# iKrishneel/fcn_object_detector

Hardware: AMD Instinct MI355X
Metric: frames/sec forward 448x448 @1 GPU; train imgs/sec @1/2/4/8 GPUs (higher is better)
Workload: dtype f32

## Files before the change

fcn_object_detector_amd/csrc/pointwise.hip:

```cpp
#include <float.h>
#include <math.h>

#include "common.h"

using namespace fcn;

namespace {

__device__ __forceinline__ float4 ld4(const float* p) { return *reinterpret_cast<const float4*>(p); }
__device__ __forceinline__ void st4(float* p, float4 v) { *reinterpret_cast<float4*>(p) = v; }

template <typename D>
__global__ __launch_bounds__(256) void nchw_to_nhwc_kernel(const float* __restrict__ src, D* __restrict__ dst,
                                                           int C, int HW, int dst_cstride, int dst_coffset, float shift) {
    __shared__ float tile[32][33];
    const int n = blockIdx.z;
    const int p0 = blockIdx.x * 32, c0 = blockIdx.y * 32;
    const int tx = threadIdx.x & 31, ty = threadIdx.x >> 5;
    const float* s = src + (size_t)n * C * HW;
    D* d = dst + (size_t)n * HW * dst_cstride;
    for (int i = ty; i < 32; i += 8) {
        const int c = c0 + i, p = p0 + tx;
        tile[i][tx] = (c < C && p < HW) ? s[(size_t)c * HW + p] : 0.f;
    }
// ... 7 lines not shown
template <typename S>
__global__ __launch_bounds__(256) void nhwc_to_nchw_kernel(const S* __restrict__ src, float* __restrict__ dst,
                                                           int C, int HW, int src_cstride, int src_coffset) {
    __shared__ float tile[32][33];
    const int n = blockIdx.z;
    const int p0 = blockIdx.x * 32, c0 = blockIdx.y * 32;
    const int tx = threadIdx.x & 31, ty = threadIdx.x >> 5;
    const S* s = src + (size_t)n * HW * src_cstride;
    float* d = dst + (size_t)n * C * HW;
    for (int i = ty; i < 32; i += 8) {
        const int p = p0 + i, c = c0 + tx;
        tile[i][tx] = (p < HW && c < C) ? (float)s[(size_t)p * src_cstride + src_coffset + c] : 0.f;
    }
    __syncthreads();
    for (int i = ty; i < 32; i += 8) {
        const int c = c0 + i, p = p0 + tx;
        if (c < C && p < HW) d[(size_t)c * HW + p] = tile[tx][i];
    }
}

__global__ __launch_bounds__(256) void nchw_to_nhwc4_kernel(const float* __restrict__ src, float* __restrict__ dst, int C, int HW, float shift) {
    const int n = blockIdx.y;
    const float* s = src + (size_t)n * C * HW;
    for (int p = blockIdx.x * blockDim.x + threadIdx.x; p < HW; p += gridDim.x * blockDim.x) {
        float4 v = make_float4(0.f, 0.f, 0.f, 0.f);
        v.x = s[p] + shift;
        if (C > 1) v.y = s[(size_t)HW + p] + shift;
        if (C > 2) v.z = s[2 * (size_t)HW + p] + shift;
        if (C > 3) v.w = s[3 * (size_t)HW + p] + shift;
        *reinterpret_cast<float4*>(dst + ((size_t)n * HW + p) * 4) = v;
    }
}

constexpr int kMaxLayoutBlobs = 8;
struct LayoutBlob { const float* src; float* dst; int C, HW, cstride, coffset, count, end; };
struct LayoutArgs { int n; LayoutBlob b[kMaxLayoutBlobs]; };
__global__ __launch_bounds__(256) void nhwc_to_nchw_multi_kernel(const LayoutArgs a) {
    const int total = a.b[a.n - 1].end;
    for (int i = blockIdx.x * blockDim.x + threadIdx.x; i < total; i += gridDim.x * blockDim.x) {
        int k = 0;
#pragma unroll
        for (int j = 0; j < kMaxLayoutBlobs - 1; ++j) k += (j + 1 < a.n && i >= a.b[j].end) ? 1 : 0;
        LayoutBlob q = a.b[0];
#pragma unroll
        for (int j = 1; j < kMaxLayoutBlobs; ++j)
            if (k == j) q = a.b[j];
        const int e = i - (q.end - q.count);
        const int p = e % q.HW, nc = e / q.HW;
        const int c = nc % q.C, n = nc / q.C;
        q.dst[e] = q.src[((size_t)n * q.HW + p) * q.cstride + q.coffset + c];
    }
}

template <bool VEC4, bool WITH_IDX>
__global__ __launch_bounds__(256) void maxpool_kernel(const float* __restrict__ x, float* __restrict__ y, int32_t* __restrict__ idx,
                                                      int N, int H, int W, int C, int x_cstride, int k, int stride, int pad,
                                                      int OH, int OW, int y_cstride, int y_coffset) {
    const int cg = VEC4 ? C / 4 : C;
    const long long total = (long long)N * OH * OW * cg;
    for (long long t = (long long)blockIdx.x * blockDim.x + threadIdx.x; t < total; t += (long long)gridDim.x * blockDim.x) {
        const int g = (int)(t % cg);
        long long pix = t / cg;
        const int ox = (int)(pix % OW);
        pix /= OW;
        const int oy = (int)(pix % OH);
        const int n = (int)(pix / OH);
        int hs = oy * stride - pad, ws = ox * stride - pad;
        const int he = min(hs + k, H), we = min(ws + k, W);
        hs = max(hs, 0);
        ws = max(ws, 0);
        const float* xb = x + (size_t)n * H * W * x_cstride + (VEC4 ? g * 4 : g);
        const size_t o = ((size_t)(n * OH + oy) * OW + ox);
        if (VEC4) {
            float4 m = make_float4(-FLT_MAX, -FLT_MAX, -FLT_MAX, -FLT_MAX);
            int4 mi = make_int4(-1, -1, -1, -1);
            if (k == 3) {
                const int y0 = oy * stride - pad, x0 = ox * stride - pad;
                float4 v[9];
                int id[9];
                bool in[9];
#pragma unroll
                for (int r = 0; r < 3; ++r) {
                    const int iy = min(max(y0 + r, 0), H - 1);
// ... 1105 lines not shown
        _Float16* dp = dst + (size_t)pix * dst_cstride + dst_coffset;
        if (!VEC) {
            dp[c] = sp[c];
        } else if (c * 8 + 8 <= C) {
            *(h8_t*)(dp + c * 8) = *(const h8_t*)(sp + c * 8);
        } else {
            const h8_t v = *(const h8_t*)(sp + c * 8);
#pragma unroll
            for (int e = 0; e < 7; ++e)
                if (c * 8 + e < C) dp[c * 8 + e] = v[e];
        }
    }
}

extern "C" {

int fcn_nchw_to_nhwc_f32(const float* src, float* dst, int N, int C, int H, int W, int dst_cstride, int dst_coffset, float shift,
                         fcn_stream_t s) {
    FCN_REQUIRE(src && dst && N > 0 && C > 0 && H > 0 && W > 0, FCN_E_ARG, "nchw_to_nhwc: bad args");
    FCN_REQUIRE(dst_coffset >= 0 && dst_cstride >= dst_coffset + C, FCN_E_ARG, "nchw_to_nhwc: slice exceeds dst_cstride");
    FCN_REQUIRE(N <= 65535, FCN_E_UNSUPPORTED, "nchw_to_nhwc: batch too large");
    const int HW = H * W;
    if (C <= 4 && dst_cstride == 4 && dst_coffset == 0 && ((uintptr_t)dst & 15) == 0) {
        hipLaunchKernelGGL(nchw_to_nhwc4_kernel, dim3(cdiv(HW, 256) < 4096 ? cdiv(HW, 256) : 4096, N), dim3(256), 0, as_stream(s), src, dst, C, HW, shift);
        FCN_LAUNCH_CHECK("nchw_to_nhwc4");
        return 0;
    }
    dim3 grid(cdiv(HW, 32), cdiv(C, 32), N);
    hipLaunchKernelGGL(nchw_to_nhwc_kernel<float>, grid, dim3(256), 0, as_stream(s), src, dst, C, HW, dst_cstride, dst_coffset, shift);
    FCN_LAUNCH_CHECK("nchw_to_nhwc");
    return 0;
}

int fcn_nhwc_to_nchw_multi_f32(const fcn_layout_desc* h_descs, int n, fcn_stream_t s) {
    FCN_REQUIRE(h_descs && n > 0 && n <= kMaxLayoutBlobs, FCN_E_ARG, "nhwc_to_nchw_multi: 1..%d blobs", kMaxLayoutBlobs);
    LayoutArgs a;
    a.n = n;
    long long end = 0;
    for (int i = 0; i < kMaxLayoutBlobs; ++i) {
        const fcn_layout_desc& d = h_descs[i < n ? i : n - 1];
        if (i < n) {
            FCN_REQUIRE(d.src && d.dst && d.N > 0 && d.C > 0 && d.H > 0 && d.W > 0, FCN_E_ARG, "nhwc_to_nchw_multi: bad blob %d", i);
            FCN_REQUIRE(d.src_coffset >= 0 && d.src_cstride >= d.src_coffset + d.C, FCN_E_ARG, "nhwc_to_nchw_multi: slice of blob %d exceeds its stride", i);
            end += (long long)d.N * d.C * d.H * d.W;
            FCN_REQUIRE(end < (1ll << 30), FCN_E_UNSUPPORTED, "nhwc_to_nchw_multi: meant for small blobs");
        }
        LayoutBlob& b = a.b[i];
        b.src = d.src; b.dst = d.dst; b.C = d.C; b.HW = d.H * d.W; b.cstride = d.src_cstride; b.coffset = d.src_coffset;
        b.count = i < n ? d.N * d.C * d.H * d.W : 0;
        b.end = (int)end;
    }
    const int blocks = cdiv(end, 256) < 2048 ? cdiv(end, 256) : 2048;
    hipLaunchKernelGGL(nhwc_to_nchw_multi_kernel, dim3(blocks), dim3(256), 0, as_stream(s), a);
    FCN_LAUNCH_CHECK("nhwc_to_nchw_multi");
    return 0;
}

int fcn_nchw_f32_to_nhwc_f16(const float* src, void* dst, int N, int C, int H, int W, int dst_cstride, int dst_coffset, float shift,
                             fcn_stream_t s) {
    FCN_REQUIRE(src && dst && N > 0 && C > 0 && H > 0 && W > 0, FCN_E_ARG, "nchw_to_nhwc_f16: bad args");
    FCN_REQUIRE(dst_coffset >= 0 && dst_cstride >= dst_coffset + C, FCN_E_ARG, "nchw_to_nhwc_f16: slice exceeds dst_cstride");
    FCN_REQUIRE(N <= 65535, FCN_E_UNSUPPORTED, "nchw_to_nhwc_f16: batch too large");
    const int HW = H * W;
    dim3 grid(cdiv(HW, 32), cdiv(C, 32), N);
    hipLaunchKernelGGL(nchw_to_nhwc_kernel<_Float16>, grid, dim3(256), 0, as_stream(s), src, reinterpret_cast<_Float16*>(dst), C, HW, dst_cstride,
                       dst_coffset, shift);
    FCN_LAUNCH_CHECK("nchw_to_nhwc_f16");
    return 0;
}

int fcn_nhwc_f16_to_nchw_f32(const void* src, float* dst, int N, int C, int H, int W, int src_cstride, int src_coffset, fcn_stream_t s) {
    FCN_REQUIRE(src && dst && N > 0 && C > 0 && H > 0 && W > 0, FCN_E_ARG, "nhwc_f16_to_nchw: bad args");
    FCN_REQUIRE(src_coffset >= 0 && src_cstride >= src_coffset + C, FCN_E_ARG, "nhwc_f16_to_nchw: slice exceeds src_cstride");
    FCN_REQUIRE(N <= 65535, FCN_E_UNSUPPORTED, "nhwc_f16_to_nchw: batch too large");
    const int HW = H * W;
    dim3 grid(cdiv(HW, 32), cdiv(C, 32), N);
    hipLaunchKernelGGL(nhwc_to_nchw_kernel<_Float16>, grid, dim3(256), 0, as_stream(s), reinterpret_cast<const _Float16*>(src), dst, C, HW,
                       src_cstride, src_coffset);
    FCN_LAUNCH_CHECK("nhwc_f16_to_nchw");
    return 0;
}

int fcn_nhwc_to_nchw_f32(const float* src, float* dst, int N, int C, int H, int W, int src_cstride, int src_coffset, fcn_stream_t s) {
    FCN_REQUIRE(src && dst && N > 0 && C > 0 && H > 0 && W > 0, FCN_E_ARG, "nhwc_to_nchw: bad args");
    FCN_REQUIRE(src_coffset >= 0 && src_cstride >= src_coffset + C, FCN_E_ARG, "nhwc_to_nchw: slice exceeds src_cstride");
    FCN_REQUIRE(N <= 65535, FCN_E_UNSUPPORTED, "nhwc_to_nchw: batch too large");
    const int HW = H * W;
// ... 412 lines not shown
```

fcn_object_detector_amd/csrc/runtime.hip:

```cpp
#include <stdarg.h>

#include "common.h"

namespace fcn {

char* err_buf() {
    static thread_local char buf[512] = {0};
    return buf;
}

int set_err(int code, const char* fmt, ...) {
    va_list ap;
    va_start(ap, fmt);
    vsnprintf(err_buf(), 512, fmt, ap);
    va_end(ap);
    return code;
}

}

using namespace fcn;

extern "C" {

// ... 20 lines not shown
    FCN_HIP(hipGetDevice(&dev));
    hipDeviceProp_t prop;
    FCN_HIP(hipGetDeviceProperties(&prop, dev));
    snprintf(h_buf, len, "%s (%s, %d CUs)", prop.name, prop.gcnArchName, prop.multiProcessorCount);
    return 0;
}

int fcn_device_sync(void) {
    FCN_HIP(hipDeviceSynchronize());
    return 0;
}

int fcn_malloc(void** p, size_t bytes) {
    FCN_REQUIRE(p, FCN_E_ARG, "fcn_malloc: null");
    if (bytes == 0) bytes = 16;
    FCN_HIP(hipMalloc(p, bytes));
    return 0;
}

int fcn_free(void* p) {
    if (p) FCN_HIP(hipFree(p));
    return 0;
}

int fcn_host_malloc(void** h_p, size_t bytes) {
    FCN_REQUIRE(h_p, FCN_E_ARG, "fcn_host_malloc: null");
    if (bytes == 0) bytes = 16;
    FCN_HIP(hipHostMalloc(h_p, bytes, hipHostMallocDefault));
    return 0;
}

int fcn_host_free(void* h_p) {
    if (h_p) FCN_HIP(hipHostFree(h_p));
    return 0;
}

int fcn_memset_async(void* p, int value, size_t bytes, fcn_stream_t s) {
    FCN_REQUIRE(p || bytes == 0, FCN_E_ARG, "fcn_memset_async: null");
    if (bytes) FCN_HIP(hipMemsetAsync(p, value, bytes, as_stream(s)));
    return 0;
}

int fcn_memcpy_h2d_async(void* dst, const void* h_src, size_t bytes, fcn_stream_t s) {
    FCN_REQUIRE((dst && h_src) || bytes == 0, FCN_E_ARG, "fcn_memcpy_h2d_async: null");
    if (bytes) FCN_HIP(hipMemcpyAsync(dst, h_src, bytes, hipMemcpyHostToDevice, as_stream(s)));
    return 0;
}

int fcn_memcpy_d2h_async(void* h_dst, const void* src, size_t bytes, fcn_stream_t s) {
    FCN_REQUIRE((h_dst && src) || bytes == 0, FCN_E_ARG, "fcn_memcpy_d2h_async: null");
    if (bytes) FCN_HIP(hipMemcpyAsync(h_dst, src, bytes, hipMemcpyDeviceToHost, as_stream(s)));
    return 0;
}

int fcn_memcpy_d2d_async(void* dst, const void* src, size_t bytes, fcn_stream_t s) {
    FCN_REQUIRE((dst && src) || bytes == 0, FCN_E_ARG, "fcn_memcpy_d2d_async: null");
    if (bytes) FCN_HIP(hipMemcpyAsync(dst, src, bytes, hipMemcpyDeviceToDevice, as_stream(s)));
    return 0;
}

int fcn_stream_create(fcn_stream_t* s) {
    FCN_REQUIRE(s, FCN_E_ARG, "fcn_stream_create: null");
    hipStream_t st;
    FCN_HIP(hipStreamCreateWithFlags(&st, hipStreamNonBlocking));
    *s = st;
    return 0;
// ... 80 lines not shown
```

fcn_object_detector_amd/engine.py:

```python
from __future__ import annotations

import ctypes as C
import os
import threading
from typing import Callable, Dict, List, Optional, Sequence, Tuple

import numpy as np

from . import lib as L
from .netspec import Layer, NetSpec, kernel_stride_pad

F32 = np.float32


def _r4(c: int) -> int:
    return (c + 3) // 4 * 4


def _ra(c: int, esize: int) -> int:
    eps = 16 // esize
    return (c + eps - 1) // eps * eps


class DeviceBuffer:
# ... 9 lines not shown

    def free(self) -> None:
        if getattr(self, "ptr", 0):
            try:
                L.load().fcn_free(self.ptr)
            finally:
                self.ptr = 0

    def __del__(self):
        try:
            self.free()
        except Exception:
            pass


class DevView:

    __slots__ = ("ptr", "nbytes")

    def __init__(self, ptr: int, nbytes: int):
        self.ptr, self.nbytes = int(ptr), int(nbytes)


class PinnedArray:

    def __init__(self, shape: Tuple[int, ...]):
        n = int(np.prod(shape)) if len(shape) else 1
        p = C.c_void_p()
        L.call("fcn_host_malloc", C.byref(p), max(n, 1) * 4)
        self.ptr = int(p.value)
        buf = (C.c_float * max(n, 1)).from_address(self.ptr)
        self.array = np.frombuffer(buf, dtype=F32, count=n).reshape(shape)
        self.array[...] = 0

    def free(self) -> None:
        if getattr(self, "ptr", 0):
            self.array = None
            try:
                L.load().fcn_host_free(self.ptr)
            finally:
                self.ptr = 0

    def __del__(self):
        try:
            self.free()
        except Exception:
            pass


class Blob:

    def __init__(self, name: str, shape: Tuple[int, ...]):
        self.name = name
        self.shape = tuple(shape)
        self.buf: Optional[DeviceBuffer] = None
        self.coffset = 0
        self.cstride = 0
        self.esize = 4
        self.lazy_shift = 0.0
        self.upload_shift = 0.0
        self.host: Optional[np.ndarray] = None
        self.pinned: Optional[PinnedArray] = None
        self.host_valid = False
        self.is_input = False

    @property
# ... 32 lines not shown
                 share_params: Optional["Engine"] = None, score_outputs: bool = False):
        if dtype not in ("f32", "f16"):
            raise ValueError("dtype must be 'f32' or 'f16'")
        if share_params is not None and (dtype != "f32" or share_params.f16):
            raise NotImplementedError("share_params: only between float32 engines (a half-float engine packs its weights differently)")
        self._share_from = share_params
        self.shared_layers: set = set()
        self.score_outputs = bool(score_outputs)
        self.score_acc: Dict[str, DeviceBuffer] = {}
        self.graph_score: Optional[int] = None
        if dtype == "f16" and spec.phase != "TEST":
            raise NotImplementedError("the half-float path is inference only (BASELINE configs[4])")
        self.dtype, self.f16 = dtype, dtype == "f16"
        self.spec = spec
        self.device = device
        self.fuse = fuse
        self.group_convs = group_convs
        self.autotune = autotune
        self._chosen_cfgs: Dict[str, int] = {}
        self._tune_from = tune_from
        self._tune_max_lds = int(tune_max_lds_kb if tune_max_lds_kb is not None else os.environ.get("FCN_TUNE_MAX_LDS_KB", "160")) * 1024
        self._tune_streams = int(tune_streams if tune_streams is not None else os.environ.get("FCN_TUNE_STREAMS", "1"))
        L.call("fcn_init", device)
        sp = C.c_void_p()
        L.call("fcn_stream_create", C.byref(sp))
        self.stream = int(sp.value)
        self.lock = threading.RLock()
        self.shapes = spec.infer(data_shapes)
        self.blobs: Dict[str, Blob] = {}
        self.params_host: Dict[str, List[np.ndarray]] = {}
        self.params_dev: Dict[str, List[DevView]] = {}
        self.ops: List[Op] = []
        self.graph_io: Optional[int] = None
        self.graph_core: Optional[int] = None
        self._staging: Dict[str, DeviceBuffer] = {}
        self._keep: List[object] = []
        self._conv_layer_meta: Dict[str, dict] = {}
        self._group_workspaces: List[DeviceBuffer] = []
        self.aux_dev: Dict[str, DeviceBuffer] = {}
        self._lazy_blob_ops: Dict[str, List[Op]] = {}
        self.loss_blobs: Dict[str, float] = {}
        self.device_fed: set = set()
        self.dropout_seed = 0
        self.dropout_index_offset = 0
        self.inputs = spec.data_tops()
        self.outputs = [b for b in spec.output_blobs() if b in self.shapes]
        self._plan_buffers()
        self._alloc_params(params)
        self._build_ops()
        self._release_tuning_resources()

    def _plan_buffers(self) -> None:
        spec = self.spec
        producers: Dict[str, List[Layer]] = {}
        consumers: Dict[str, List[Layer]] = {}
        for l in spec.layers:
            for t in l.tops:
                producers.setdefault(t, []).append(l)
            for b in l.bottoms:
                consumers.setdefault(b, []).append(l)
        self.producers, self.consumers = producers, consumers
        data_tops = set(self.inputs)
        self._half_inputs: Dict[str, Tuple[str, float]] = {}
        if self.f16 and self.fuse and os.environ.get("FCN_F16_IMAGE", "1") != "0":
            for d in data_tops:
                cons = consumers.get(d, [])
# ... 1124 lines not shown
                out.append(Op("tconv", l.name, lambda st: L.check(lib.fcn_tconv2d_f32(C.byref(plan), st)),
                              2.0 * n * h * w * c * co * k * k, 4.0 * (xb.pixels * c + yb.pixels * co)))
                return out
            if halves:
                if xb.esize != 2 or xb.coffset % 8:
                    raise NotImplementedError("f16 engine: Deconvolution %s from a float32 blob / an unaligned channel slice" % l.name)
                out.append(Op("deconv", l.name, lambda st: L.check(lib.fcn_deconv_depthwise_fwd_f16(
                    xb.ptr, wdev, bdev, yb.buf.ptr, n, h, w, c, xb.cstride, k, s, pad, oh, ow, yb.cstride, yb.coffset,
                    1 if yb.esize == 4 else 0, st)),
                    2.0 * yb.pixels * c * (k / s) ** 2, float(xb.esize * xb.pixels + yb.esize * yb.pixels) * c))
                return out
            out.append(Op("deconv", l.name, lambda st: L.check(lib.fcn_deconv_depthwise_fwd_f32(
                xb.ptr, wdev, bdev, yb.buf.ptr, n, h, w, c, xb.cstride, k, s, pad, oh, ow, yb.cstride, yb.coffset, st)),
                2.0 * yb.pixels * c * (k / s) ** 2, 4.0 * (xb.pixels + yb.pixels) * c))
        else:
            raise NotImplementedError("layer type %r (layer %s) has no forward kernel yet" % (t, l.name))
        return out

    def _stage(self, name: str) -> DeviceBuffer:
        st = self._staging.get(name)
        if st is None:
            b = self.blobs[name]
            st = DeviceBuffer(max(int(np.prod(b.shape)) if b.shape else 1, 1) * 4, zero=False)
            self._staging[name] = st
        return st

    def host_array(self, name: str) -> np.ndarray:
        b = self.blobs[name]
        if b.host is None:
            b.pinned = PinnedArray(b.shape)
            b.host = b.pinned.array
        return b.host

    def _upload_copy(self, name: str, stream: Optional[int]) -> None:
        b = self.blobs[name]
        host = self.host_array(name)
        dst = b.ptr if len(b.shape) != 4 else self._stage(name).ptr
        L.check(L.load().fcn_memcpy_h2d_async(dst, host.ctypes.data, host.nbytes, stream))

    def _upload_convert(self, name: str, stream: Optional[int]) -> None:
        b = self.blobs[name]
        if len(b.shape) != 4:
            return
        lib = L.load()
        n, c, h, w = b.shape
        st = self._stage(name)
        if b.esize == 2:
            L.check(lib.fcn_nchw_f32_to_nhwc_f16(st.ptr, b.buf.ptr, n, c, h, w, b.cstride, b.coffset, b.upload_shift, stream))
        else:
            L.check(lib.fcn_nchw_to_nhwc_f32(st.ptr, b.buf.ptr, n, c, h, w, b.cstride, b.coffset, b.upload_shift, stream))

    def _download_convert(self, name: str, stream: Optional[int]) -> None:
        b = self.blobs[name]
        if len(b.shape) != 4:
            return
        lib = L.load()
        n, c, h, w = b.shape
        st = self._stage(name)
        if b.esize == 2:
            L.check(lib.fcn_nhwc_f16_to_nchw_f32(b.buf.ptr, st.ptr, n, c, h, w, b.cstride, b.coffset, stream))
        else:
            L.check(lib.fcn_nhwc_to_nchw_f32(b.buf.ptr, st.ptr, n, c, h, w, b.cstride, b.coffset, stream))

    def _download_convert_all(self, stream: Optional[int]) -> None:
        multi = [nm for nm in self.outputs if len(self.blobs[nm].shape) == 4 and self.blobs[nm].esize == 4]
        if 2 <= len(multi) <= 8:
            if not hasattr(self, "_multi_descs"):
                arr = (L.LayoutDesc * len(multi))()
                for d, nm in zip(arr, multi):
                    b = self.blobs[nm]
                    n, c, h, w = b.shape
                    d.src, d.dst, d.N, d.C, d.H, d.W, d.src_cstride, d.src_coffset = b.buf.ptr, self._stage(nm).ptr, n, c, h, w, b.cstride, b.coffset
                self._multi_descs = arr
            L.check(L.load().fcn_nhwc_to_nchw_multi_f32(self._multi_descs, len(multi), stream))
        else:
            multi = []
        for nm in self.outputs:
            if nm not in multi:
                self._download_convert(nm, stream)

    def _download_copy(self, name: str, stream: Optional[int]) -> None:
        b = self.blobs[name]
        host = self.host_array(name)
        src = b.ptr if len(b.shape) != 4 else self._stage(name).ptr
        L.check(L.load().fcn_memcpy_d2h_async(host.ctypes.data, src, host.nbytes, stream))

    def _enqueue_upload(self, name: str, stream: Optional[int]) -> None:
        self._upload_copy(name, stream)
        self._upload_convert(name, stream)

    def _enqueue_download(self, name: str, stream: Optional[int]) -> None:
        self._download_convert(name, stream)
        self._download_copy(name, stream)

    def read_blob(self, name: str) -> np.ndarray:
        with self.lock:
            L.call("fcn_init", self.device)
            b = self.blobs[name]
            host = self.host_array(name)
            if not b.host_valid:
                for op in self._lazy_blob_ops.get(name, ()):
                    op.run(self.stream)
                self._enqueue_download(name, self.stream)
                L.call("fcn_stream_sync", self.stream)
                if b.lazy_shift:
                    host += F32(b.lazy_shift)
                b.host_valid = True
            return host

    LABEL_TOPS = ("coverage-label", "bbox-label", "size-block", "obj-block", "coverage-block")

    def set_targets(self, rects: Sequence[Sequence[Sequence[int]]], labels: Sequence[Sequence[int]], stride: int,
                    iou_thresh: float = 0.1, tops: Sequence[str] = LABEL_TOPS) -> None:
        fg = self.blobs[tops[0]]
# ... 66 lines not shown
            if self.graph_score is not None:
                L.call("fcn_graph_launch", self.graph_score, self.stream)
            else:
                for nm in self.inputs:
                    if nm not in self.device_fed:
                        self._upload_convert(nm, self.stream)
                self.run_ops(self.stream)
            for b in self.blobs.values():
                b.host_valid = False
            self.score_forwards += 1

    def score_read(self) -> Dict[str, np.ndarray]:
        with self.lock:
            out = {nm: np.empty(self.blobs[nm].shape, F32) for nm in self.outputs}
            for nm, a in out.items():
                L.call("fcn_memcpy_d2h_async", a.ctypes.data, self.score_acc[nm].ptr, a.nbytes, self.stream)
            L.call("fcn_stream_sync", self.stream)
            return out

    def run_ops(self, stream: Optional[int]) -> None:
        for op in self.ops:
            op.run(stream)

    def _capture(self, with_io: bool, download: bool = True) -> int:
        if with_io:
            for nm in list(self.inputs) + list(self.outputs):
                self.host_array(nm)
                if len(self.blobs[nm].shape) == 4:
                    self._stage(nm)
        if not getattr(self, "_warm", False):
            self.run_ops(self.stream)
            L.call("fcn_stream_sync", self.stream)
            self._warm = True
        if with_io and not getattr(self, "_warm_io", False):
            for nm in self.inputs:
                if nm not in self.device_fed:
                    self._enqueue_upload(nm, self.stream)
            self._download_convert_all(self.stream)
            for nm in self.outputs:
                self._download_copy(nm, self.stream)
            L.call("fcn_stream_sync", self.stream)
            self._warm_io = True
        L.call("fcn_graph_begin", self.stream)
        try:
            if with_io:
                for nm in self.inputs:
                    if nm not in self.device_fed:
                        self._upload_convert(nm, self.stream)
            self.run_ops(self.stream)
            if with_io and download:
                self._download_convert_all(self.stream)
        finally:
            g = C.c_void_p()
            L.call("fcn_graph_end", self.stream, C.byref(g))
        return int(g.value)

    def _launch_io(self) -> None:
        if self.graph_io is None:
            self.graph_io = self._capture(with_io=True)
        for nm in self.inputs:
            if nm not in self.device_fed:
                self._upload_copy(nm, self.stream)
        L.call("fcn_graph_launch", self.graph_io, self.stream)
        for nm in self.outputs:
            self._download_copy(nm, self.stream)

    def forward(self, use_graph: bool = True) -> Dict[str, np.ndarray]:
        use_graph = use_graph and os.environ.get("FCN_NO_GRAPH", "0") in ("", "0")
        with self.lock:
            L.call("fcn_init", self.device)
            for nm in self.inputs:
                self.host_array(nm)
            for nm in self.outputs:
                self.host_array(nm)
            if use_graph:
                self._launch_io()
            else:
                for nm in self.inputs:
                    if nm not in self.device_fed:
                        self._enqueue_upload(nm, self.stream)
                self.run_ops(self.stream)
                for nm in self.outputs:
                    self._enqueue_download(nm, self.stream)
            L.call("fcn_stream_sync", self.stream)
            for b in self.blobs.values():
                b.host_valid = False
            out = {}
            for nm in self.outputs:
                b = self.blobs[nm]
                if b.lazy_shift:
                    b.host += F32(b.lazy_shift)
                b.host_valid = True
                out[nm] = b.host
            for nm in self.inputs:
                self.blobs[nm].host_valid = nm not in self.device_fed
            return out

    def forward_begin(self) -> None:
# ... 256 lines not shown
```

fcn_object_detector_amd/lib.py:

```python
from __future__ import annotations

import ctypes as C
import os
import threading
from typing import Optional

_HERE = os.path.dirname(os.path.abspath(__file__))
LIB_PATH = os.environ.get("FCN_LIB_PATH") or os.path.join(_HERE, "libfcnhip.so")


class FcnLibraryError(RuntimeError):
    pass


class FcnError(RuntimeError):
    def __init__(self, code: int, msg: str):
        super().__init__("libfcnhip error %d: %s" % (code, msg))
        self.code = code


class ConvDesc(C.Structure):
    _fields_ = [
        ("x", C.c_void_p), ("w", C.c_void_p), ("bias", C.c_void_p), ("y", C.c_void_p), ("y2", C.c_void_p),
        ("N", C.c_int32), ("H", C.c_int32), ("W", C.c_int32), ("Cin", C.c_int32), ("x_cstride", C.c_int32),
# ... 58 lines not shown
    _fields_ = [("w_offset", C.c_uint64), ("wt_offset", C.c_uint64), ("Cout", C.c_int32), ("kh", C.c_int32), ("kw", C.c_int32),
                ("Cin", C.c_int32), ("Cin4", C.c_int32), ("Cout4", C.c_int32)]


class DetectParams(C.Structure):
    _fields_ = [
        ("num_classes", C.c_int32), ("gy", C.c_int32), ("gx", C.c_int32), ("cell_w", C.c_int32), ("cell_h", C.c_int32),
        ("cvg_cstride", C.c_int32), ("cvg_coffset", C.c_int32), ("box_cstride", C.c_int32), ("box_coffset", C.c_int32),
        ("prob_thresh", C.c_float), ("group_thresh", C.c_int32), ("eps", C.c_double), ("min_height", C.c_int32),
        ("round_mode", C.c_int32), ("max_out", C.c_int32),
    ]


CONV_RELU, CONV_SIGMOID2, CONV_ACCUM, CONV_OUT_F32, CONV_F16, CONV_OUT_F16, CONV_MASK = 1, 2, 4, 8, 16, 32, 64
CONV_IMAGE_ONES = 128
ELT_PROD, ELT_SUM, ELT_MAX = 0, 1, 2
SOLVER_KINDS = {"SGD": 0, "NESTEROV": 1, "ADAGRAD": 2, "RMSPROP": 3, "ADADELTA": 4, "ADAM": 5}
REG_L2, REG_L1 = 0, 1
RECT_ROUND_NEAREST_EVEN, RECT_ROUND_TRUNCATE = 0, 1

_vp, _i, _f, _d, _sz = C.c_void_p, C.c_int, C.c_float, C.c_double, C.c_size_t

PROTOTYPES = {
    "fcn_abi_version": (_i, []),
    "fcn_last_error_string": (C.c_char_p, []),
    "fcn_device_count": (_i, [C.POINTER(_i)]),
    "fcn_init": (_i, [_i]),
    "fcn_device_name": (_i, [C.c_char_p, _i]),
    "fcn_device_sync": (_i, []),
    "fcn_malloc": (_i, [C.POINTER(_vp), _sz]),
    "fcn_free": (_i, [_vp]),
    "fcn_host_malloc": (_i, [C.POINTER(_vp), _sz]),
    "fcn_host_free": (_i, [_vp]),
    "fcn_memset_async": (_i, [_vp, _i, _sz, _vp]),
    "fcn_memcpy_h2d_async": (_i, [_vp, _vp, _sz, _vp]),
    "fcn_memcpy_d2h_async": (_i, [_vp, _vp, _sz, _vp]),
    "fcn_memcpy_d2d_async": (_i, [_vp, _vp, _sz, _vp]),
    "fcn_stream_create": (_i, [C.POINTER(_vp)]),
    "fcn_stream_destroy": (_i, [_vp]),
    "fcn_stream_sync": (_i, [_vp]),
    "fcn_event_create": (_i, [C.POINTER(_vp)]),
    "fcn_event_destroy": (_i, [_vp]),
    "fcn_event_record": (_i, [_vp, _vp]),
    "fcn_event_sync": (_i, [_vp]),
    "fcn_event_elapsed_ms": (_i, [_vp, _vp, C.POINTER(_f)]),
    "fcn_graph_begin": (_i, [_vp]),
    "fcn_graph_end": (_i, [_vp, C.POINTER(_vp)]),
    "fcn_graph_launch": (_i, [_vp, _vp]),
    "fcn_graph_destroy": (_i, [_vp]),
    "fcn_nchw_to_nhwc_f32": (_i, [_vp, _vp, _i, _i, _i, _i, _i, _i, _f, _vp]),
    "fcn_nhwc_to_nchw_f32": (_i, [_vp, _vp, _i, _i, _i, _i, _i, _i, _vp]),
    "fcn_nhwc_to_nchw_multi_f32": (_i, [C.POINTER(LayoutDesc), _i, _vp]),
    "fcn_conv2d_fwd_f32": (_i, [C.POINTER(ConvDesc), _vp]),
    "fcn_conv2d_group_workspace_bytes": (_sz, [_i]),
    "fcn_conv2d_num_configs": (_i, []),
    "fcn_conv2d_first_layer_config": (_i, []),
    "fcn_conv2d_config_lds_bytes": (_i, [_i]),
    "fcn_conv2d_config_waves_k": (_i, [_i]),
    "fcn_conv2d_group_prepare": (_i, [C.POINTER(ConvDesc), _i, _vp, _i, C.POINTER(ConvGroup)]),
    "fcn_conv2d_group_prepare_fused": (_i, [C.POINTER(ConvDesc), _i, C.POINTER(PoolDesc), _i, _vp, _i, C.POINTER(ConvGroup)]),
    "fcn_conv2d_fwd_group_f32": (_i, [C.POINTER(ConvGroup), _vp]),
    "fcn_conv2d_group_release": (_i, [_vp]),
    "fcn_conv2d_tail_scratch_bytes": (C.c_size_t, [C.POINTER(ConvTail)]),
    "fcn_conv2d_tail_arrive_bytes": (C.c_size_t, [C.POINTER(ConvTail)]),
    "fcn_conv2d_group_attach_tail": (_i, [_vp, C.POINTER(ConvTail)]),
    "fcn_maxpool_fwd_f32": (_i, [_vp, _vp, _vp] + [_i] * 12 + [_vp]),
    "fcn_avepool_fwd_f32": (_i, [_vp, _vp] + [_i] * 12 + [_vp]),
    "fcn_lrn_fwd_f32": (_i, [_vp, _vp, _vp, _i, _i, _i, _i, _i, _f, _f, _f, _vp]),
    "fcn_maxpool_lrn5_fwd_f32": (_i, [_vp, _vp] + [_i] * 12 + [_f, _f, _f, _vp]),
    "fcn_maxpool_lrn5_fwd_f16": (_i, [_vp, _vp] + [_i] * 12 + [_f, _f, _f, _vp]),
    "fcn_maxpool_lrn5_conv1x1_fwd_f32": (_i, [_vp] + [_i] * 10 + [_f, _f, _f, _vp, _vp, _i, _i, _vp, _i, _i, _vp]),
    "fcn_maxpool_lrn5_conv1x1_fwd_f16": (_i, [_vp] + [_i] * 10 + [_f, _f, _f, _vp, _vp, _i, _i, _vp, _i, _i, _vp]),
    "fcn_relu_fwd_f32": (_i, [_vp, _vp, _sz, _f, _vp]),
    "fcn_sigmoid_fwd_f32": (_i, [_vp, _vp, _sz, _vp]),
    "fcn_power_fwd_f32": (_i, [_vp, _vp, _sz, _f, _f, _f, _vp]),
    "fcn_eltwise_fwd_f32": (_i, [_vp, _vp, _vp, _sz, _i, _f, _f, _vp]),
    "fcn_copy_channels_f32": (_i, [_vp, _vp, _i, _i, _i, _i, _i, _i, _vp]),
    "fcn_deconv_depthwise_fwd_f32": (_i, [_vp, _vp, _vp, _vp] + [_i] * 12 + [_vp]),
    "fcn_preprocess_bgr8": (_i, [_vp, _i, _i, _vp, _i, _i, _i, _f, _vp, _vp]),
    "fcn_detect_workspace_bytes": (_sz, [C.POINTER(DetectParams), _i]),
    "fcn_detect_decode_group": (_i, [_vp, _vp, _i, _sz, _sz, C.POINTER(DetectParams), _vp, _vp, _vp, _vp, _vp]),
    "fcn_score_masks_workspace_bytes": (_sz, [_i, _i, _i, _i]),
    "fcn_score_masks": (_i, [_vp, _i, _i, _i, _i, _i, _i, _vp, _f, _vp, _i, _i, _vp, _vp, _vp]),
    "fcn_gen_targets": (_i, [_vp, _vp, _vp, _i, _i, _i, _i, _i, _d, _vp, _vp, _vp, _vp, _vp, _vp]),
    "fcn_gen_targets_nhwc": (_i, [_vp, _vp, _vp, _i, _i, _i, _i, _i, _d, _vp, _i, _vp, _vp, _vp, _vp, _i, _vp]),
# ... 119 lines not shown
```

include/fcnhip.h:

```cpp
#ifndef FCNHIP_H_
#define FCNHIP_H_

#include <stddef.h>
#include <stdint.h>

#ifdef __cplusplus
extern "C" {
#endif

#define FCN_ABI_VERSION 1

#define FCN_E_ARG       1
#define FCN_E_ALIGN     2
#define FCN_E_UNSUPPORTED 3
#define FCN_E_STATE     4
#define FCN_E_CAPACITY  5

typedef void* fcn_stream_t;
typedef void* fcn_event_t;
typedef void* fcn_graph_t;
typedef void* fcn_comm_t;

int  fcn_abi_version(void);
const char* fcn_last_error_string(void);
int  fcn_device_count(int* count);
int  fcn_init(int device);
int  fcn_device_name(char* h_buf, int len);
int  fcn_device_sync(void);
int  fcn_malloc(void** p, size_t bytes);
int  fcn_free(void* p);
int  fcn_host_malloc(void** h_p, size_t bytes);
int  fcn_host_free(void* h_p);
int  fcn_memset_async(void* p, int value, size_t bytes, fcn_stream_t s);
int  fcn_memcpy_h2d_async(void* dst, const void* h_src, size_t bytes, fcn_stream_t s);
int  fcn_memcpy_d2h_async(void* h_dst, const void* src, size_t bytes, fcn_stream_t s);
int  fcn_memcpy_d2d_async(void* dst, const void* src, size_t bytes, fcn_stream_t s);
int  fcn_stream_create(fcn_stream_t* s);
int  fcn_stream_destroy(fcn_stream_t s);
int  fcn_stream_sync(fcn_stream_t s);
int  fcn_event_create(fcn_event_t* e);
int  fcn_event_destroy(fcn_event_t e);
int  fcn_event_record(fcn_event_t e, fcn_stream_t s);
int  fcn_event_sync(fcn_event_t e);
int  fcn_event_elapsed_ms(fcn_event_t start, fcn_event_t stop, float* h_ms);
int  fcn_stream_wait_event(fcn_stream_t s, fcn_event_t e);
int  fcn_graph_begin(fcn_stream_t s);
int  fcn_graph_end(fcn_stream_t s, fcn_graph_t* g);
int  fcn_graph_launch(fcn_graph_t g, fcn_stream_t s);
int  fcn_graph_destroy(fcn_graph_t g);

int  fcn_nchw_to_nhwc_f32(const float* src, float* dst, int N, int C, int H, int W,
                          int dst_cstride, int dst_coffset, float shift, fcn_stream_t s);
int  fcn_nhwc_to_nchw_f32(const float* src, float* dst, int N, int C, int H, int W,
                          int src_cstride, int src_coffset, fcn_stream_t s);
typedef struct fcn_layout_desc {
    const float* src;
    float* dst;
    int32_t N, C, H, W, src_cstride, src_coffset;
} fcn_layout_desc;
int  fcn_nhwc_to_nchw_multi_f32(const fcn_layout_desc* h_descs, int n, fcn_stream_t s);

#define FCN_CONV_RELU      1
#define FCN_CONV_SIGMOID2  2
#define FCN_CONV_ACCUM     4
#define FCN_CONV_MASK     64
#define FCN_CONV_IMAGE_ONES 128
#define FCN_CONV_OUT_F32   8
#define FCN_CONV_OUT_F16  32
#define FCN_CONV_F16      16
typedef struct fcn_conv_desc {
    const float* x;
    const float* w;
    const float* bias;
    float*       y;
    float*       y2;
    int32_t N, H, W, Cin, x_cstride;
    int32_t Cout, kh, kw, pad, stride, OH, OW;
    int32_t y_cstride, y_coffset, y2_cstride, y2_coffset;
    int32_t flags;
    float   in_shift;
} fcn_conv_desc;
int  fcn_conv2d_fwd_f32(const fcn_conv_desc* h_desc, fcn_stream_t s);
typedef struct fcn_conv_group {
    void*   d_probs;
    int32_t n;
    int32_t cfg;
    int32_t total_tiles;
} fcn_conv_group;
size_t fcn_conv2d_group_workspace_bytes(int n);
int  fcn_conv2d_num_configs(void);
int  fcn_conv2d_first_layer_config(void);
typedef struct fcn_conv_tail {
    int32_t n;
// ... 243 lines not shown
```

Baseline: 4237.

## Write outputs directly into pinned host memory via zero-copy kernels

Adds zero-copy I/O. The layout-conversion kernels now read the input frame from, or write outputs into, mapped pinned host memory through device pointers. This removes the separate staging buffers and the d2h/h2d memcpy steps around the captured graph. Output stores to host memory use nontemporal writes, with blob starts padded to 64 elements, and an optional vectorised host-read input kernel uses a small grid. The risk is that PCIe-latency-bound kernel stores run inside the graph and could slow it, and that the graph must be recaptured if the pinned buffers change.

```diff
diff --git a/fcn_object_detector_amd/csrc/pointwise.hip b/fcn_object_detector_amd/csrc/pointwise.hip
--- a/fcn_object_detector_amd/csrc/pointwise.hip
+++ b/fcn_object_detector_amd/csrc/pointwise.hip
@@ -63,23 +63,60 @@
     }
 }
 
+constexpr int kHostGroups = 2;
+constexpr int kHostGridMax = 64;
+typedef float f32x4 __attribute__((ext_vector_type(4)));
+template <int C>
+__global__ __launch_bounds__(256) void nchw_to_nhwc4_from_host_kernel(const float* __restrict__ src, float* __restrict__ dst, int HW, float shift) {
+    const int n = blockIdx.y;
+    const int groups = HW / 4, stride = gridDim.x * blockDim.x;
+    const f32x4* s = reinterpret_cast<const f32x4*>(src + (size_t)n * C * HW);
+    f32x4* d = reinterpret_cast<f32x4*>(dst + (size_t)n * HW * 4);
+    for (int g0 = blockIdx.x * blockDim.x + threadIdx.x; g0 < groups; g0 += stride * kHostGroups) {
+        f32x4 v[kHostGroups][C];
+#pragma unroll
+        for (int u = 0; u < kHostGroups; ++u) {
+            const int g = g0 + u * stride;
+#pragma unroll
+            for (int c = 0; c < C; ++c) v[u][c] = g < groups ? __builtin_nontemporal_load(s + (size_t)c * groups + g) : f32x4{0.f, 0.f, 0.f, 0.f};
+        }
+#pragma unroll
+        for (int u = 0; u < kHostGroups; ++u) {
+            const int g = g0 + u * stride;
+            if (g < groups) {
+#pragma unroll
+                for (int j = 0; j < 4; ++j) {
+                    f32x4 o = {0.f, 0.f, 0.f, 0.f};
+#pragma unroll
+                    for (int c = 0; c < C; ++c) o[c] = v[u][c][j] + shift;
+                    d[(size_t)g * 4 + j] = o;
+                }
+            }
+        }
+    }
+}
+
 constexpr int kMaxLayoutBlobs = 8;
-struct LayoutBlob { const float* src; float* dst; int C, HW, cstride, coffset, count, end; };
+struct LayoutBlob { const float* src; float* dst; int C, HW, cstride, coffset, start, end; };
 struct LayoutArgs { int n; LayoutBlob b[kMaxLayoutBlobs]; };
+template <bool TO_HOST>
 __global__ __launch_bounds__(256) void nhwc_to_nchw_multi_kernel(const LayoutArgs a) {
     const int total = a.b[a.n - 1].end;
     for (int i = blockIdx.x * blockDim.x + threadIdx.x; i < total; i += gridDim.x * blockDim.x) {
         int k = 0;
 #pragma unroll
-        for (int j = 0; j < kMaxLayoutBlobs - 1; ++j) k += (j + 1 < a.n && i >= a.b[j].end) ? 1 : 0;
+        for (int j = 0; j < kMaxLayoutBlobs - 1; ++j) k += (j + 1 < a.n && i >= a.b[j + 1].start) ? 1 : 0;
         LayoutBlob q = a.b[0];
 #pragma unroll
         for (int j = 1; j < kMaxLayoutBlobs; ++j)
             if (k == j) q = a.b[j];
-        const int e = i - (q.end - q.count);
+        if (i >= q.end) continue;
+        const int e = i - q.start;
         const int p = e % q.HW, nc = e / q.HW;
         const int c = nc % q.C, n = nc / q.C;
-        q.dst[e] = q.src[((size_t)n * q.HW + p) * q.cstride + q.coffset + c];
+        const float v = q.src[((size_t)n * q.HW + p) * q.cstride + q.coffset + c];
+        if (TO_HOST) __builtin_nontemporal_store(v, q.dst + e);
+        else q.dst[e] = v;
     }
 }
 
@@ -1251,27 +1288,54 @@
     return 0;
 }
 
-int fcn_nhwc_to_nchw_multi_f32(const fcn_layout_desc* h_descs, int n, fcn_stream_t s) {
+static int nhwc_to_nchw_multi(const fcn_layout_desc* h_descs, int n, bool to_host, fcn_stream_t s) {
     FCN_REQUIRE(h_descs && n > 0 && n <= kMaxLayoutBlobs, FCN_E_ARG, "nhwc_to_nchw_multi: 1..%d blobs", kMaxLayoutBlobs);
     LayoutArgs a;
     a.n = n;
     long long end = 0;
     for (int i = 0; i < kMaxLayoutBlobs; ++i) {
         const fcn_layout_desc& d = h_descs[i < n ? i : n - 1];
+        LayoutBlob& b = a.b[i];
+        b.src = d.src; b.dst = d.dst; b.C = d.C; b.HW = d.H * d.W; b.cstride = d.src_cstride; b.coffset = d.src_coffset;
+        if (to_host) end = (end + 63) / 64 * 64;
+        b.start = (int)end;
         if (i < n) {
             FCN_REQUIRE(d.src && d.dst && d.N > 0 && d.C > 0 && d.H > 0 && d.W > 0, FCN_E_ARG, "nhwc_to_nchw_multi: bad blob %d", i);
             FCN_REQUIRE(d.src_coffset >= 0 && d.src_cstride >= d.src_coffset + d.C, FCN_E_ARG, "nhwc_to_nchw_multi: slice of blob %d exceeds its stride", i);
             end += (long long)d.N * d.C * d.H * d.W;
             FCN_REQUIRE(end < (1ll << 30), FCN_E_UNSUPPORTED, "nhwc_to_nchw_multi: meant for small blobs");
         }
-        LayoutBlob& b = a.b[i];
-        b.src = d.src; b.dst = d.dst; b.C = d.C; b.HW = d.H * d.W; b.cstride = d.src_cstride; b.coffset = d.src_coffset;
-        b.count = i < n ? d.N * d.C * d.H * d.W : 0;
         b.end = (int)end;
     }
     const int blocks = cdiv(end, 256) < 2048 ? cdiv(end, 256) : 2048;
-    hipLaunchKernelGGL(nhwc_to_nchw_multi_kernel, dim3(blocks), dim3(256), 0, as_stream(s), a);
+    if (to_host) hipLaunchKernelGGL(nhwc_to_nchw_multi_kernel<true>, dim3(blocks), dim3(256), 0, as_stream(s), a);
+    else hipLaunchKernelGGL(nhwc_to_nchw_multi_kernel<false>, dim3(blocks), dim3(256), 0, as_stream(s), a);
     FCN_LAUNCH_CHECK("nhwc_to_nchw_multi");
+    return 0;
+}
+
+int fcn_nhwc_to_nchw_multi_f32(const fcn_layout_desc* h_descs, int n, fcn_stream_t s) { return nhwc_to_nchw_multi(h_descs, n, false, s); }
+
+int fcn_nhwc_to_nchw_multi_f32_to_host(const fcn_layout_desc* h_descs, int n, fcn_stream_t s) { return nhwc_to_nchw_multi(h_descs, n, true, s); }
+
+int fcn_nchw_to_nhwc_f32_from_host(const float* src, float* dst, int N, int C, int H, int W, int dst_cstride, int dst_coffset, float shift,
+                                   fcn_stream_t s) {
+    FCN_REQUIRE(src && dst && N > 0 && C > 0 && H > 0 && W > 0, FCN_E_ARG, "nchw_to_nhwc_from_host: bad args");
+    FCN_REQUIRE(dst_coffset >= 0 && dst_cstride >= dst_coffset + C, FCN_E_ARG, "nchw_to_nhwc_from_host: slice exceeds dst_cstride");
+    FCN_REQUIRE(N <= 65535, FCN_E_UNSUPPORTED, "nchw_to_nhwc_from_host: batch too large");
+    const int HW = H * W;
+    if (!(C <= 4 && dst_cstride == 4 && dst_coffset == 0 && HW % 4 == 0 && (((uintptr_t)src | (uintptr_t)dst) & 15) == 0))
+        return fcn_nchw_to_nhwc_f32(src, dst, N, C, H, W, dst_cstride, dst_coffset, shift, s);
+    int blocks = cdiv(HW / 4, 256 * kHostGroups);
+    if (blocks > kHostGridMax) blocks = cdiv(blocks, cdiv(blocks, kHostGridMax));
+    const dim3 grid(blocks, N);
+    switch (C) {
+        case 1: hipLaunchKernelGGL(nchw_to_nhwc4_from_host_kernel<1>, grid, dim3(256), 0, as_stream(s), src, dst, HW, shift); break;
+        case 2: hipLaunchKernelGGL(nchw_to_nhwc4_from_host_kernel<2>, grid, dim3(256), 0, as_stream(s), src, dst, HW, shift); break;
+        case 3: hipLaunchKernelGGL(nchw_to_nhwc4_from_host_kernel<3>, grid, dim3(256), 0, as_stream(s), src, dst, HW, shift); break;
+        default: hipLaunchKernelGGL(nchw_to_nhwc4_from_host_kernel<4>, grid, dim3(256), 0, as_stream(s), src, dst, HW, shift); break;
+    }
+    FCN_LAUNCH_CHECK("nchw_to_nhwc4_from_host");
     return 0;
 }
 
diff --git a/fcn_object_detector_amd/csrc/runtime.hip b/fcn_object_detector_amd/csrc/runtime.hip
--- a/fcn_object_detector_amd/csrc/runtime.hip
+++ b/fcn_object_detector_amd/csrc/runtime.hip
@@ -76,6 +76,12 @@
 
 int fcn_host_free(void* h_p) {
     if (h_p) FCN_HIP(hipHostFree(h_p));
+    return 0;
+}
+
+int fcn_host_device_ptr(void* h_p, void** d_p) {
+    FCN_REQUIRE(h_p && d_p, FCN_E_ARG, "fcn_host_device_ptr: null");
+    FCN_HIP(hipHostGetDevicePointer(d_p, h_p, 0));
     return 0;
 }
 
diff --git a/fcn_object_detector_amd/engine.py b/fcn_object_detector_amd/engine.py
--- a/fcn_object_detector_amd/engine.py
+++ b/fcn_object_detector_amd/engine.py
@@ -65,6 +65,14 @@
         buf = (C.c_float * max(n, 1)).from_address(self.ptr)
         self.array = np.frombuffer(buf, dtype=F32, count=n).reshape(shape)
         self.array[...] = 0
+        self._device_ptr = 0
+
+    def device_ptr(self) -> int:
+        if not self._device_ptr:
+            p = C.c_void_p()
+            L.call("fcn_host_device_ptr", self.ptr, C.byref(p))
+            self._device_ptr = int(p.value)
+        return self._device_ptr
 
     def free(self) -> None:
         if getattr(self, "ptr", 0):
@@ -163,6 +171,8 @@
         self.params_dev: Dict[str, List[DevView]] = {}
         self.ops: List[Op] = []
         self.graph_io: Optional[int] = None
+        self._direct: frozenset = frozenset()
+        self._graph_io_hosts: Dict[str, int] = {}
         self.graph_core: Optional[int] = None
         self._staging: Dict[str, DeviceBuffer] = {}
         self._keep: List[object] = []
@@ -1353,7 +1363,18 @@
             b.host = b.pinned.array
         return b.host
 
+    def _direct_io_names(self) -> frozenset:
+        level = os.environ.get("FCN_ZERO_COPY_IO", "1") or "0"
+        if level not in ("0", "1", "2"):
+            raise ValueError("FCN_ZERO_COPY_IO must be 0 (staged), 1 (outputs written to host memory) or 2 (and the frame read from it)")
+        plain = lambda b: len(b.shape) == 4 and b.esize == 4
+        ins = [nm for nm in self.inputs if nm not in self.device_fed and plain(self.blobs[nm])] if level == "2" else []
+        outs = [nm for nm in self.outputs if plain(self.blobs[nm]) and not self.blobs[nm].lazy_shift and nm not in self.inputs]
+        return frozenset(ins + (outs if level != "0" and len(outs) <= 8 else []))
+
     def _upload_copy(self, name: str, stream: Optional[int]) -> None:
+        if name in self._direct:
+            return
         b = self.blobs[name]
         host = self.host_array(name)
         dst = b.ptr if len(b.shape) != 4 else self._stage(name).ptr
@@ -1365,6 +1386,9 @@
             return
         lib = L.load()
         n, c, h, w = b.shape
+        if name in self._direct:
+            L.check(lib.fcn_nchw_to_nhwc_f32_from_host(b.pinned.device_ptr(), b.buf.ptr, n, c, h, w, b.cstride, b.coffset, b.upload_shift, stream))
+            return
         st = self._stage(name)
         if b.esize == 2:
             L.check(lib.fcn_nchw_f32_to_nhwc_f16(st.ptr, b.buf.ptr, n, c, h, w, b.cstride, b.coffset, b.upload_shift, stream))
@@ -1384,23 +1408,32 @@
             L.check(lib.fcn_nhwc_to_nchw_f32(b.buf.ptr, st.ptr, n, c, h, w, b.cstride, b.coffset, stream))
 
     def _download_convert_all(self, stream: Optional[int]) -> None:
-        multi = [nm for nm in self.outputs if len(self.blobs[nm].shape) == 4 and self.blobs[nm].esize == 4]
+        def descs(names, dst):
+            arr = (L.LayoutDesc * len(names))()
+            for d, nm in zip(arr, names):
+                b = self.blobs[nm]
+                n, c, h, w = b.shape
+                d.src, d.dst, d.N, d.C, d.H, d.W, d.src_cstride, d.src_coffset = b.buf.ptr, dst(nm), n, c, h, w, b.cstride, b.coffset
+            return arr
+        direct = [nm for nm in self.outputs if nm in self._direct]
+        if direct:
+            if getattr(self, "_direct_descs", None) is None:
+                self._direct_descs = descs(direct, lambda nm: self.blobs[nm].pinned.device_ptr())
+            L.check(L.load().fcn_nhwc_to_nchw_multi_f32_to_host(self._direct_descs, len(direct), stream))
+        multi = [nm for nm in self.outputs if nm not in direct and len(self.blobs[nm].shape) == 4 and self.blobs[nm].esize == 4]
         if 2 <= len(multi) <= 8:
             if not hasattr(self, "_multi_descs"):
-                arr = (L.LayoutDesc * len(multi))()
-                for d, nm in zip(arr, multi):
-                    b = self.blobs[nm]
-                    n, c, h, w = b.shape
-                    d.src, d.dst, d.N, d.C, d.H, d.W, d.src_cstride, d.src_coffset = b.buf.ptr, self._stage(nm).ptr, n, c, h, w, b.cstride, b.coffset
-                self._multi_descs = arr
+                self._multi_descs = descs(multi, lambda nm: self._stage(nm).ptr)
             L.check(L.load().fcn_nhwc_to_nchw_multi_f32(self._multi_descs, len(multi), stream))
         else:
             multi = []
         for nm in self.outputs:
-            if nm not in multi:
+            if nm not in multi and nm not in direct:
                 self._download_convert(nm, stream)
 
     def _download_copy(self, name: str, stream: Optional[int]) -> None:
+        if name in self._direct:
+            return
         b = self.blobs[name]
         host = self.host_array(name)
         src = b.ptr if len(b.shape) != 4 else self._stage(name).ptr
@@ -1533,38 +1566,54 @@
             self.run_ops(self.stream)
             L.call("fcn_stream_sync", self.stream)
             self._warm = True
-        if with_io and not getattr(self, "_warm_io", False):
+        self._direct = self._direct_io_names() if with_io and download else frozenset()
+        try:
+            for nm in self._direct:
+                self.blobs[nm].pinned.device_ptr()
+            warm = "_warm_io_direct" if self._direct else "_warm_io"
+            if with_io and not getattr(self, warm, False):
+                for nm in self.inputs:
+                    if nm not in self.device_fed:
+                        self._enqueue_upload(nm, self.stream)
+                self._download_convert_all(self.stream)
+                for nm in self.outputs:
+                    self._download_copy(nm, self.stream)
+                L.call("fcn_stream_sync", self.stream)
+                setattr(self, warm, True)
+            L.call("fcn_graph_begin", self.stream)
+            try:
+                if with_io:
+                    for nm in self.inputs:
+                        if nm not in self.device_fed:
+                            self._upload_convert(nm, self.stream)
+                self.run_ops(self.stream)
+                if with_io and download:
+                    self._download_convert_all(self.stream)
+            finally:
+                g = C.c_void_p()
+                L.call("fcn_graph_end", self.stream, C.byref(g))
+            if with_io and download:
+                self._graph_io_hosts = {nm: self.blobs[nm].pinned.ptr for nm in self._direct}
+        finally:
+            self._direct = frozenset()
+        return int(g.value)
+
+    def _launch_io(self) -> None:
+        if self.graph_io is not None and any(self.blobs[nm].pinned.ptr != p for nm, p in self._graph_io_hosts.items()):
+            L.call("fcn_graph_destroy", self.graph_io)
+            self.graph_io, self._direct_descs = None, None
+        if self.graph_io is None:
+            self.graph_io = self._capture(with_io=True)
+        self._direct = frozenset(self._graph_io_hosts)
+        try:
             for nm in self.inputs:
                 if nm not in self.device_fed:
-                    self._enqueue_upload(nm, self.stream)
-            self._download_convert_all(self.stream)
+                    self._upload_copy(nm, self.stream)
+            L.call("fcn_graph_launch", self.graph_io, self.stream)
             for nm in self.outputs:
                 self._download_copy(nm, self.stream)
-            L.call("fcn_stream_sync", self.stream)
-            self._warm_io = True
-        L.call("fcn_graph_begin", self.stream)
-        try:
-            if with_io:
-                for nm in self.inputs:
-                    if nm not in self.device_fed:
-                        self._upload_convert(nm, self.stream)
-            self.run_ops(self.stream)
-            if with_io and download:
-                self._download_convert_all(self.stream)
         finally:
-            g = C.c_void_p()
-            L.call("fcn_graph_end", self.stream, C.byref(g))
-        return int(g.value)
-
-    def _launch_io(self) -> None:
-        if self.graph_io is None:
-            self.graph_io = self._capture(with_io=True)
-        for nm in self.inputs:
-            if nm not in self.device_fed:
-                self._upload_copy(nm, self.stream)
-        L.call("fcn_graph_launch", self.graph_io, self.stream)
-        for nm in self.outputs:
-            self._download_copy(nm, self.stream)
+            self._direct = frozenset()
 
     def forward(self, use_graph: bool = True) -> Dict[str, np.ndarray]:
         use_graph = use_graph and os.environ.get("FCN_NO_GRAPH", "0") in ("", "0")
diff --git a/fcn_object_detector_amd/lib.py b/fcn_object_detector_amd/lib.py
--- a/fcn_object_detector_amd/lib.py
+++ b/fcn_object_detector_amd/lib.py
@@ -114,6 +114,7 @@
     "fcn_free": (_i, [_vp]),
     "fcn_host_malloc": (_i, [C.POINTER(_vp), _sz]),
     "fcn_host_free": (_i, [_vp]),
+    "fcn_host_device_ptr": (_i, [_vp, C.POINTER(_vp)]),
     "fcn_memset_async": (_i, [_vp, _i, _sz, _vp]),
     "fcn_memcpy_h2d_async": (_i, [_vp, _vp, _sz, _vp]),
     "fcn_memcpy_d2h_async": (_i, [_vp, _vp, _sz, _vp]),
@@ -133,6 +134,8 @@
     "fcn_nchw_to_nhwc_f32": (_i, [_vp, _vp, _i, _i, _i, _i, _i, _i, _f, _vp]),
     "fcn_nhwc_to_nchw_f32": (_i, [_vp, _vp, _i, _i, _i, _i, _i, _i, _vp]),
     "fcn_nhwc_to_nchw_multi_f32": (_i, [C.POINTER(LayoutDesc), _i, _vp]),
+    "fcn_nchw_to_nhwc_f32_from_host": (_i, [_vp, _vp, _i, _i, _i, _i, _i, _i, _f, _vp]),
+    "fcn_nhwc_to_nchw_multi_f32_to_host": (_i, [C.POINTER(LayoutDesc), _i, _vp]),
     "fcn_conv2d_fwd_f32": (_i, [C.POINTER(ConvDesc), _vp]),
     "fcn_conv2d_group_workspace_bytes": (_sz, [_i]),
     "fcn_conv2d_num_configs": (_i, []),
diff --git a/include/fcnhip.h b/include/fcnhip.h
--- a/include/fcnhip.h
+++ b/include/fcnhip.h
@@ -31,6 +31,7 @@
 int  fcn_free(void* p);
 int  fcn_host_malloc(void** h_p, size_t bytes);
 int  fcn_host_free(void* h_p);
+int  fcn_host_device_ptr(void* h_p, void** d_p);
 int  fcn_memset_async(void* p, int value, size_t bytes, fcn_stream_t s);
 int  fcn_memcpy_h2d_async(void* dst, const void* h_src, size_t bytes, fcn_stream_t s);
 int  fcn_memcpy_d2h_async(void* h_dst, const void* src, size_t bytes, fcn_stream_t s);
@@ -59,6 +60,9 @@
     int32_t N, C, H, W, src_cstride, src_coffset;
 } fcn_layout_desc;
 int  fcn_nhwc_to_nchw_multi_f32(const fcn_layout_desc* h_descs, int n, fcn_stream_t s);
+int  fcn_nchw_to_nhwc_f32_from_host(const float* src, float* dst, int N, int C, int H, int W,
+                                    int dst_cstride, int dst_coffset, float shift, fcn_stream_t s);
+int  fcn_nhwc_to_nchw_multi_f32_to_host(const fcn_layout_desc* h_descs, int n, fcn_stream_t s);
 
 #define FCN_CONV_RELU      1
 #define FCN_CONV_SIGMOID2  2
```

Result: no change. 4255 (median of 6 runs) (+0.4%).
